# ofsouzap/DistributedMandelbrot

Hardware: AMD Instinct MI355X
Metric: G pixel-iterations/s on 4096^2 tile, max_iter=1000 fp64 (higher is better)
Workload: dtype f64

## Files before the change

distributedmandelbrot_amd/_lib.py:

```python
from __future__ import annotations

import ctypes as C
import importlib.util
import os
import sys

HERE = os.path.dirname(os.path.abspath(__file__))
SO_PATH = os.path.join(HERE, "libmbk_hip.so")

MBK_OK, MBK_ERR_INVALID, MBK_ERR_NO_DEVICE, MBK_ERR_HIP, MBK_ERR_NOMEM, MBK_ERR_NET = range(6)
MBK_WANT_COUNTS = 0x1
MBK_WANT_BYTES = 0x2
MBK_KERNEL_DEFAULT = 0x000
MBK_KERNEL_SIMPLE = 0x100
MBK_KERNEL_ASM = 0x200
MBK_KERNEL_REFILL = 0x300
MBK_KERNEL_GROUP = 0x400
MBK_KERNEL_SCAN = 0x500
KERNELS = {"default": MBK_KERNEL_DEFAULT, "simple": MBK_KERNEL_SIMPLE, "asm": MBK_KERNEL_ASM,
           "refill": MBK_KERNEL_REFILL, "group": MBK_KERNEL_GROUP, "scan": MBK_KERNEL_SCAN}
OPTIONS = {name: i for i, name in enumerate(
    ["order", "waves_per_wg", "group_steps", "exact_steps", "probe_steps", "scan_waves", "scan_xcd_map", "scan_col_period", "heavy_share",
     "rf_livemin", "rf_patience", "rf_batch", "rf_waves", "cycle_detect", "probe_mid", "prepass_overlap", "exact_long", "scan_inline", "wave_limit", "units_min_light", "xcd_balance", "m_late", "h_settled", "classify_wg", "scan_strip", "cycle_window", "spill_first", "spill_lanes", "spill_min_mrd", "spill_min_blocks", "spill_cyc_shift",
     "sure_interior"])}
MBK_PRECISION_F32 = 0x1000
MBK_LAZY_UNIFORM = 0x2000
MBK_DEEP_BLA = 0x8000
MBK_DEEP_XBLA = 0x10000
PRECISIONS = {"f64": 0, "f32": MBK_PRECISION_F32}
MBK_SLOTS = 4
MBK_WORKER_DEPTH = 3
MBK_INFO_SCAN_WG_PER_CU = 100
MBK_INFO_XCD_SHARE = 110
MBK_INFO_SPILL = 130
MBK_CODEC_RAW = 0x00
MBK_CODEC_RLE = 0x01
MBK_CHUNK_DEFINITION = 4096
MBK_CHUNK_BYTES = 4096 * 4096
MBK_ABI_VERSION = 5
MBK_RENDER_BYTES = 0
MBK_RENDER_SMOOTH = 1
MBK_RENDER_DISTANCE = 3
MBK_RENDER_DISTANCE_REL = 4
MBK_RENDER_EQUALIZED = 5
RENDER_SOURCES = {"bytes": MBK_RENDER_BYTES, "smooth": MBK_RENDER_SMOOTH, "distance": MBK_RENDER_DISTANCE,
                  "distance_rel": MBK_RENDER_DISTANCE_REL, "equalized": MBK_RENDER_EQUALIZED}
MBK_HISTOGRAM_MAX_MRD = 1 << 20
# ... 131 lines not shown
    "mbk_view_launch_distance": (C.c_int, [C.c_void_p, C.POINTER(mbk_view), C.c_uint32, C.c_uint32,
                                           C.c_void_p, C.c_void_p, C.c_void_p]),
    "mbk_view_compute_distance": (C.c_int, [C.c_void_p, C.POINTER(mbk_view), C.c_uint32, C.c_uint32,
                                            C.c_void_p, C.c_void_p, C.POINTER(mbk_stats)]),
    "mbk_distance_value_host": (C.c_double, [C.c_double, C.c_double, C.c_int32]),
    "mbk_datachunk_submit": (C.c_int, [C.c_void_p, C.c_int, C.c_uint32, C.c_uint32, C.c_uint32, C.c_uint32,
                                       C.c_void_p, C.c_void_p]),
    "mbk_datachunk_submit_ex": (C.c_int, [C.c_void_p, C.c_int, C.c_uint32, C.c_uint32, C.c_uint32, C.c_uint32,
                                          C.c_void_p, C.c_void_p, C.c_uint32]),
    "mbk_view_submit": (C.c_int, [C.c_void_p, C.c_int, C.POINTER(mbk_view), C.c_uint32, C.c_uint32,
                                  C.c_void_p, C.c_void_p]),
    "mbk_wait": (C.c_int, [C.c_void_p, C.c_int, C.POINTER(mbk_stats)]),
    "mbk_serialize_last": (C.c_int, [C.c_void_p, C.c_void_p, C.c_uint64, C.POINTER(C.c_uint64),
                                     C.POINTER(C.c_uint32)]),
    "mbk_set_option": (C.c_int, [C.c_void_p, C.c_int, C.c_uint32]),
    "mbk_get_option": (C.c_int, [C.c_void_p, C.c_int, C.POINTER(C.c_uint32)]),
    "mbk_quantise_counts": (C.c_int, [C.c_void_p, C.c_void_p, C.c_uint64, C.c_uint32, C.c_void_p]),
    "mbk_units_plan": (C.c_int, [C.c_uint32, C.c_uint32, C.c_uint32, C.c_void_p, C.c_void_p]),
    "mbk_units_lookup": (C.c_int, [C.c_void_p, C.c_uint32, C.c_void_p, C.c_void_p]),
    "mbk_sure_interior_point": (C.c_int, [C.c_double, C.c_double]),
    "mbk_sure_interior_blocks": (C.c_int, [C.POINTER(mbk_view), C.POINTER(C.c_uint64)]),
    "mbk_sure_interior_flag": (C.c_int, [C.POINTER(mbk_view), C.c_uint32, C.c_uint32, C.c_uint32, C.c_uint32,
                                         C.POINTER(C.c_uint32)]),
    "mbk_reduce_counts": (C.c_int, [C.c_void_p, C.c_void_p, C.c_uint64, C.c_uint32, C.c_void_p,
                                    C.POINTER(mbk_stats)]),
    "mbk_worker_run": (C.c_int, [C.c_void_p, C.c_char_p, C.c_uint16, C.c_uint64, C.c_uint32,
                                 C.POINTER(mbk_worker_report)]),
    "mbk_net_set_option": (C.c_int, [C.c_int, C.c_uint32]),
    "mbk_net_get_option": (C.c_int, [C.c_int, C.POINTER(C.c_uint32)]),
    "mbk_feeder_run": (C.c_int, [C.POINTER(mbk_feeder_ops), C.c_char_p, C.c_uint16, C.c_uint64, C.c_uint32,
                                 C.POINTER(mbk_worker_report)]),
    "mbk_deep_orbit_create": (C.c_int, [C.c_char_p, C.c_char_p, C.c_uint32, C.c_uint32, C.POINTER(C.c_void_p)]),
    "mbk_deep_orbit_destroy": (None, [C.c_void_p]),
    "mbk_deep_orbit_info": (C.c_int, [C.c_void_p, C.POINTER(C.c_uint32), C.POINTER(C.c_uint32), C.POINTER(C.c_uint32),
                                      C.POINTER(C.c_uint32)]),
    "mbk_deep_orbit_read": (C.c_int, [C.c_void_p, C.c_void_p, C.c_void_p, C.c_uint64]),
    "mbk_deep_view_launch": (C.c_int, [C.c_void_p, C.c_void_p, C.POINTER(mbk_deep_view), C.c_uint32, C.c_uint32,
                                       C.c_void_p, C.c_void_p, C.c_void_p, C.c_void_p]),
    "mbk_deep_view_compute": (C.c_int, [C.c_void_p, C.c_void_p, C.POINTER(mbk_deep_view), C.c_uint32, C.c_uint32,
                                        C.c_void_p, C.c_void_p, C.c_void_p, C.POINTER(mbk_stats)]),
    "mbk_deep_view_submit": (C.c_int, [C.c_void_p, C.c_int, C.c_void_p, C.POINTER(mbk_deep_view), C.c_uint32, C.c_uint32,
                                       C.c_void_p, C.c_void_p]),
    "mbk_deep_view_launch_distance": (C.c_int, [C.c_void_p, C.c_void_p, C.POINTER(mbk_deep_view), C.c_uint32, C.c_uint32,
                                                C.c_void_p, C.c_void_p, C.c_void_p]),
    "mbk_deep_view_compute_distance": (C.c_int, [C.c_void_p, C.c_void_p, C.POINTER(mbk_deep_view), C.c_uint32, C.c_uint32,
                                                 C.c_void_p, C.c_void_p, C.POINTER(mbk_stats)]),
# ... 287 lines not shown
```

distributedmandelbrot_amd/csrc/mbk_api.hip:

```cpp
#include "../../include/mbk.h"

#include <hip/hip_runtime.h>

#include <cmath>
#include <cstdio>
#include <cstdlib>
#include <algorithm>
#include <cstring>
#include <new>
#include <string>
#include <vector>

#include "mbk_kernels.h"
#include "mbk_refill.h"
#include "mbk_persist.h"
#include "mbk_scan.h"
#include "mbk_units.h"
#include "mbk_spill.h"
#include "mbk_feeder.h"
#include "mbk_deep_orbit.h"
#include "mbk_deep.h"
#include "mbk_deep_bla.h"
#include "mbk_deep_wide.h"
#include "mbk_deep_wide_bla.h"
// ... 371 lines not shown
}

static int get_scratch(mbk_ctx *ctx, hipStream_t stream, StreamScratch **out)
{
    for (StreamScratch &sc : ctx->scratch)
        if (sc.stream == stream) {
            *out = &sc;
            return MBK_OK;
        }
    if (ctx->scratch.size() >= kMaxStreamScratch) {
        MBK_HIP(ctx, hipDeviceSynchronize());
        for (StreamScratch &sc : ctx->scratch) free_scratch(sc);
        ctx->scratch.clear();
    }
    ctx->scratch.emplace_back();
    StreamScratch &sc = ctx->scratch.back();
    sc.stream = stream;
    *out = &sc;
    MBK_HIP(ctx, hipHostMalloc((void **)&sc.h_hint, 2 * sizeof(uint32_t), hipHostMallocDefault));
    sc.h_hint[0] = sc.h_hint[1] = 0xffffffffu;
    return MBK_OK;
}

static void set_window_facts(TileArgs &a, bool f32, bool cyc = true, uint32_t sure_option = 0u);
static void shares_from_fractions(const double *f, uint32_t *cum);
static double window_heavy_share(const TileArgs &a);
static double window_heavy_share(mbk_ctx *ctx, const TileArgs &a);

static void xcd_shares_update(const mbk_ctx *ctx, StreamScratch &sc)
{
    const unsigned long long kMask = 0xffffffffffffull;
    uint32_t first = sc.xcd_issued >= kStampSlots ? sc.xcd_issued - kStampSlots + 1u : 1u;
    first = std::max(first, sc.xcd_consumed + 1u);
    for (uint32_t c = first; c <= sc.xcd_issued; ++c) {
        const volatile unsigned long long *st = sc.h_stamps + (size_t)(c % kStampSlots) * mbk::kStampWords;
        const StreamScratch::SharesUsed &used = sc.xcd_ring[c % kShareRing];
        if (used.seq != c) continue;
        const StreamScratch::SharesUsed &before = sc.xcd_ring[(c - 1u) % kShareRing], &after = sc.xcd_ring[(c + 1u) % kShareRing];
        const bool alone = c > 1u && before.seq == c - 1u && before.switches == used.switches &&
                           (c == sc.xcd_issued ? ctx->stream_switches == used.switches : after.seq == c + 1u && after.switches == used.switches);
        unsigned long long v[mbk::kStampWords];
        bool whole = true;
        for (uint32_t i = 0; i < mbk::kStampWords; ++i) {
            v[i] = st[i];
            whole = whole && (v[i] >> 48) == (c & 0xffffu);
        }
        if (!whole) continue;
// ... 31 lines not shown
{
    uint32_t qtab = 0u;
    if (want_bytes && mrd > 0)
        for (uint32_t c = 1; c <= 4u; ++c)
            qtab |= (uint32_t)(((uint64_t)c * 256u + (uint32_t)mrd - 1u) / (uint32_t)mrd & 0xffu) << (8u * (c - 1u));
    return qtab;
}

struct BlockLaunchPlan {
    uint32_t wpw, by;
    dim3 grid, block;
    uint32_t order_mode, probe_steps;
    bool cyc, units, ordered;
    double unit_share;
};

static BlockLaunchPlan block_launch_plan(mbk_ctx *ctx, TileArgs &a, uint32_t kernel, bool safe, bool f32)
{
    BlockLaunchPlan p;
    p.wpw = ctx->opt[MBK_OPT_WAVES_PER_WG];
    a.blocks_x = (a.ncols + 8u * p.wpw - 1u) / (8u * p.wpw);
    p.by = (a.nrows + 7u) / 8u;
    p.cyc = ctx->opt[MBK_OPT_CYCLE_DETECT] != 0u;
    set_window_facts(a, f32, p.cyc, ctx->opt[MBK_OPT_SURE_INTERIOR]);
    p.grid = dim3(a.blocks_x * p.by);
    p.block = dim3(64u * p.wpw);
    p.order_mode = ctx->opt[MBK_OPT_ORDER];
    p.probe_steps = ctx->opt[MBK_OPT_PROBE_STEPS];
    a.perm_mul = p.order_mode == 1 ? coprime_multiplier(p.grid.x) : 1u;
    a.order = nullptr;
    p.units = p.order_mode == 3 && p.wpw == 1u && kernel == MBK_KERNEL_GROUP && !safe && a.smooth == nullptr &&
              (a.counts || a.bytes) && !(a.bytes && a.quant_wide) && a.blocks_x % 8u == 0u && a.blocks_x <= 2048u &&
              a.fast_bx_end > 0u && a.fast_by_end > 0u && (f32 || ctx->opt[MBK_OPT_GROUP_STEPS] == 16u) &&
              p.grid.x >= 16384u && (uint32_t)a.mrd > 2u * p.probe_steps && p.by <= 0xffffu;
    p.unit_share = 0.0;
    if (p.units) {
        p.unit_share = window_heavy_share(ctx, a);
        p.units = (1.0 - p.unit_share) * 65536.0 >= (double)ctx->opt[MBK_OPT_UNITS_MIN_LIGHT];
    }
    p.ordered = p.order_mode >= 2 && p.grid.x >= 16384u && (uint32_t)a.mrd > 2u * p.probe_steps && a.blocks_x <= 0xffffu && p.by <= 0xffffu;
    return p;
}

struct OrderList {
    StreamScratch *sc = nullptr;
    unsigned k = 0;
    uint32_t *list = nullptr;
// ... 279 lines not shown
        MBK_HIP(ctx, hipEventRecord(ol.sc->ring.ev_done[ol.k], stream));
        ol.sc->ring.done_valid[ol.k] = true;
    }
    if (spill) {
        const int rc = enqueue_spill_second_pass(ctx, a, *spill, p.grid.x, f32, p.cyc, stream);
        if (rc != MBK_OK) return rc;
    }
    ol.whole = true;
    return MBK_OK;
}

static bool window_may_touch_ring(const TileArgs &a, double margin = 1e-6)
{
    const double x0 = axis_value_host(a.re, a.col0), x1 = axis_value_host(a.re, a.col0 + a.ncols - 1u);
    const double y0 = axis_value_host(a.im, a.row0), y1 = axis_value_host(a.im, a.row0 + a.nrows - 1u);
    const double xlo = std::fmin(x0, x1), xhi = std::fmax(x0, x1), ylo = std::fmin(y0, y1), yhi = std::fmax(y0, y1);
    const double dx = (xlo <= 0.0 && 0.0 <= xhi) ? 0.0 : std::fmin(std::fabs(xlo), std::fabs(xhi));
    const double dy = (ylo <= 0.0 && 0.0 <= yhi) ? 0.0 : std::fmin(std::fabs(ylo), std::fabs(yhi));
    const double fx = std::fmax(std::fabs(xlo), std::fabs(xhi)), fy = std::fmax(std::fabs(ylo), std::fabs(yhi));
    const double rmin2 = dx * dx + dy * dy, rmax2 = fx * fx + fy * fy;
    return !(rmax2 < 4.0 - margin || rmin2 > 4.0 + margin);
}

static uint32_t sure_interior_word(const TileArgs &a, bool f32, bool cyc, uint32_t option)
{
    if (option == 0u || f32 || cyc || a.mrd < 65) return 0u;
    if (option == 2u) return 2u;
    if (a.ncols == 0u || a.nrows == 0u) return 0u;
    const double x0 = axis_value_host(a.re, a.col0), x1 = axis_value_host(a.re, a.col0 + a.ncols - 1u);
    const double y0 = axis_value_host(a.im, a.row0), y1 = axis_value_host(a.im, a.row0 + a.nrows - 1u);
    const double xlo = std::fmin(x0, x1), xhi = std::fmax(x0, x1), ylo = std::fmin(y0, y1), yhi = std::fmax(y0, y1);
    if (!(xlo <= 0.4 && xhi >= -1.3 && ylo <= 0.7 && yhi >= -0.7)) return 0u;
    const uint32_t k = 16;
    for (uint32_t j = 0; j < k; ++j) {
        const double ci = axis_value_host(a.im, a.row0 + (uint32_t)(((uint64_t)(2u * j + 1u) * a.nrows) / (2u * k)));
        for (uint32_t i = 0; i < k; ++i)
            if (mbk::sure_interior_point(axis_value_host(a.re, a.col0 + (uint32_t)(((uint64_t)(2u * i + 1u) * a.ncols) / (2u * k))), ci))
                return 1u;
    }
    return 0u;
}

static void set_window_facts(TileArgs &a, bool f32, bool cyc, uint32_t sure_option)
{
    a.sure_interior = sure_interior_word(a, f32, cyc, sure_option);
    a.ring_possible = window_may_touch_ring(a, f32 ? 2e-3 : 1e-6) ? 1u : 0u;
    a.fast_bx_end = a.fast_by_end = 0u;
    if (a.re.step_is_zero || a.im.step_is_zero) return;
    const uint64_t re_n = (uint64_t)a.re.n - (axis_end_is_regular(a.re) ? 0u : 1u), im_n = (uint64_t)a.im.n - (axis_end_is_regular(a.im) ? 0u : 1u);
    const uint64_t cols_ok = std::min<uint64_t>(a.ncols, re_n - std::min<uint64_t>(a.col0, re_n));
    const uint64_t rows_ok = std::min<uint64_t>(a.nrows, im_n - std::min<uint64_t>(a.row0, im_n));
    a.fast_bx_end = (uint32_t)(cols_ok / 8u);
    a.fast_by_end = (uint32_t)(rows_ok / 8u);
}

static int launch_refill(mbk_ctx *ctx, const TileArgs &a, bool safe, hipStream_t stream)
{
    const bool eligible = !safe && a.mrd >= 2 && a.counts != nullptr && !a.re.step_is_zero &&
                          !a.im.step_is_zero && !window_may_touch_ring(a, 1e-6);
    const uint32_t cols_ok = a.re.n > 0 ? std::min<uint64_t>(a.ncols, (uint64_t)(a.re.n - 1u) - std::min<uint64_t>(a.col0, a.re.n - 1u)) : 0u;
    const uint32_t rows_ok = a.im.n > 0 ? std::min<uint64_t>(a.nrows, (uint64_t)(a.im.n - 1u) - std::min<uint64_t>(a.row0, a.im.n - 1u)) : 0u;
    const uint32_t icols = eligible ? (cols_ok / 8u) * 8u : 0u, irows = eligible ? (rows_ok / 8u) * 8u : 0u;
    if (icols == 0 || irows == 0) return launch_blocks(ctx, a, MBK_KERNEL_GROUP, safe, false, stream);

    mbk::PersistArgs q;
    std::memset(&q, 0, sizeof(q));
    q.re_start = a.re.start;
    q.re_step = a.re.step;
// ... 710 lines not shown
}

int mbk_create(int device, mbk_ctx **out)
{
    if (!out) return fail(nullptr, MBK_ERR_INVALID, "out is NULL");
    *out = nullptr;
    int n = 0;
    hipError_t e = hipGetDeviceCount(&n);
    if (e != hipSuccess || n <= 0)
        return fail(nullptr, MBK_ERR_NO_DEVICE,
                    std::string("no HIP device visible (") + hipGetErrorString(e) +
                        "); libmbk_hip has no CPU fallback");
    if (device < 0 || device >= n) return fail(nullptr, MBK_ERR_NO_DEVICE, "device index out of range");
    mbk_ctx *ctx = new (std::nothrow) mbk_ctx();
    if (!ctx) return fail(nullptr, MBK_ERR_NOMEM, "out of host memory");
    ctx->device = device;
    static const uint32_t kDefaults[MBK_OPT_COUNT_] = {
         3u,  1u,  16u,  8u,  32u,
         8u,  1u,  4u,  655u,
         48u,  256u,  1u,  8u,  1u,
         65537u,  1u,  0u,  1u,  0u,
         32768u,  0u,  8u,  6u,  1024u,
         1u,  32u,  256u,  16u,  2048u,  19u,  5u,
         1u};
    std::memcpy(ctx->opt, kDefaults, sizeof(kDefaults));
#define MBK_CREATE_HIP(call)                                                        \
    do {                                                                            \
        hipError_t e2_ = (call);                                                    \
        if (e2_ != hipSuccess) {                                                    \
            fail(nullptr, MBK_ERR_HIP, std::string(#call) + ": " + hipGetErrorString(e2_)); \
            mbk_destroy(ctx);                                                       \
            return MBK_ERR_HIP;                                                     \
        }                                                                           \
    } while (0)
    MBK_CREATE_HIP(hipSetDevice(device));
    MBK_CREATE_HIP(hipGetDeviceProperties(&ctx->prop, device));
    if (std::strncmp(ctx->prop.gcnArchName, "gfx950", 6) != 0) {
        fail(nullptr, MBK_ERR_NO_DEVICE,
             std::string("device is ") + ctx->prop.gcnArchName + ", this library is built for gfx950 only");
        mbk_destroy(ctx);
        return MBK_ERR_NO_DEVICE;
    }
    for (Slot &sl : ctx->s) {
        MBK_CREATE_HIP(hipStreamCreateWithFlags(&sl.stream, hipStreamNonBlocking));
        MBK_CREATE_HIP(hipEventCreate(&sl.ev_k0));
        MBK_CREATE_HIP(hipEventCreate(&sl.ev_k1));
        MBK_CREATE_HIP(hipEventCreate(&sl.ev_c0));
// ... 638 lines not shown
        case MBK_OPT_RF_LIVEMIN: ok = value <= 63u; break;
        case MBK_OPT_RF_PATIENCE: ok = value >= 16u && value <= (1u << 20); break;
        case MBK_OPT_RF_BATCH: ok = value >= 1u && value <= 64u; break;
        case MBK_OPT_RF_WAVES: ok = value >= 1u && value <= 8u; break;
        case MBK_OPT_CYCLE_DETECT: ok = value <= 1u; break;
        case MBK_OPT_PROBE_MID: ok = value >= 2u && value <= 65537u; break;
        case MBK_OPT_PREPASS_OVERLAP: ok = value <= 2u; break;
        case MBK_OPT_CLASSIFY_WG: ok = value >= 64u && value <= 1024u && value % 64u == 0u; break;
        case MBK_OPT_SCAN_STRIP: ok = value <= 1u; break;
        case MBK_OPT_CYCLE_WINDOW: ok = value <= 65536u; break;
        case MBK_OPT_EXACT_LONG: ok = value <= 4096u; break;
        case MBK_OPT_SCAN_INLINE: ok = value <= 1u; break;
        case MBK_OPT_WAVE_LIMIT: ok = value <= 7u; break;
        case MBK_OPT_UNITS_MIN_LIGHT: ok = value <= 65536u; break;
        case MBK_OPT_XCD_BALANCE: ok = value <= 2u; break;
        case MBK_OPT_M_LATE: ok = value <= 65536u; break;
        case MBK_OPT_H_SETTLED: ok = value <= 30u; break;
        case MBK_OPT_SPILL_FIRST: ok = value <= 65536u && value % 32u == 0u; break;
        case MBK_OPT_SPILL_LANES: ok = value >= 1u && value <= 32u; break;
        case MBK_OPT_SPILL_MIN_MRD: ok = true; break;
        case MBK_OPT_SPILL_MIN_BLOCKS: ok = value <= 31u; break;
        case MBK_OPT_SPILL_CYC_SHIFT: ok = value <= 31u; break;
        case MBK_OPT_SURE_INTERIOR: ok = value <= 2u; break;
        default: return fail(ctx, MBK_ERR_INVALID, "unknown MBK_OPT_* selector");
    }
    if (!ok) return fail(ctx, MBK_ERR_INVALID, "option value out of range");
    ctx->opt[option] = value;
    return MBK_OK;
}

int mbk_get_option(mbk_ctx *ctx, int option, uint32_t *value)
{
    if (!ctx || !value) return fail(ctx, MBK_ERR_INVALID, "NULL argument");
    if (option >= MBK_INFO_SCAN_WG_PER_CU && option < MBK_INFO_SCAN_WG_PER_CU + 4) {
        const int k = option - MBK_INFO_SCAN_WG_PER_CU;
        *value = (uint32_t)ctx->scan_occ[k >> 1][k & 1];
        return MBK_OK;
    }
    if (option >= MBK_INFO_XCD_SHARE && option < MBK_INFO_XCD_SHARE + 10) {
        const StreamScratch *best = nullptr;
        for (const StreamScratch &sc : ctx->scratch)
            if (!best || sc.xcd_consumed > best->xcd_consumed) best = &sc;
        const int k = option - MBK_INFO_XCD_SHARE;
        *value = !best ? 0u : k < 8 ? (uint32_t)std::lround(best->xcd_f[k] * 1048576.0) : k == 8 ? best->xcd_consumed : best->xcd_issued;
        return MBK_OK;
    }
// ... 68 lines not shown
            for (uint32_t ly = 0; ly < 8u && all; ++ly) {
                const double ci = (double)(a.row0 + by * 8u + ly) * a.im.step + a.im.start;
                for (uint32_t lx = 0; lx < 8u && all; ++lx)
                    all = mbk::sure_interior_point((double)(a.col0 + bx * 8u + lx) * a.re.step + a.re.start, ci);
            }
            n += all ? 1u : 0u;
        }
    *certified = n;
    return MBK_OK;
}

int mbk_sure_interior_flag(const mbk_view *view, uint32_t mrd, uint32_t flags, uint32_t cycle_detect, uint32_t option, uint32_t *flag)
{
    if (!view || !flag) return fail(nullptr, MBK_ERR_INVALID, "NULL argument");
    if (option > 2u || mrd > 0x7fffffffu) return fail(nullptr, MBK_ERR_INVALID, "option value out of range");
    const bool f32 = (flags & MBK_PRECISION_F32) != 0;
    bool safe = false;
    const int rc = validate_view(nullptr, view, &safe, f32);
    if (rc != MBK_OK) return rc;
    TileArgs a = view_window_args(view);
    a.mrd = (int32_t)mrd;
    set_window_facts(a, f32, cycle_detect != 0u, option);
    *flag = a.sure_interior;
    return MBK_OK;
}

int mbk_quantise_counts(mbk_ctx *ctx, const int32_t *h_counts, uint64_t n, uint32_t mrd, uint8_t *h_bytes)
{
    if (!ctx || !h_counts || !h_bytes) return fail(ctx, MBK_ERR_INVALID, "NULL argument");
    if (mrd == 0 || mrd > 0x7fffffffu) return fail(ctx, MBK_ERR_INVALID, "mrd must be in [1, 2^31)");
    if (n == 0) return MBK_OK;
    if (n > (1ull << 31)) return fail(ctx, MBK_ERR_INVALID, "more than 2^31 counts");
    int rc = sync_begin(ctx);
    if (rc != MBK_OK) return rc;
    Slot &sl = ctx->s[0];
    rc = ensure_buffers(ctx, sl, (size_t)n);
    if (rc != MBK_OK) return rc;
    MBK_HIP(ctx, hipMemcpyAsync(sl.d_counts, h_counts, n * sizeof(int32_t), hipMemcpyHostToDevice, sl.stream));
    hipLaunchKernelGGL(mbk::quantise_kernel, dim3(2048), dim3(256), 0, sl.stream, sl.d_counts, sl.d_bytes, n,
                       (int32_t)mrd, mrd >= (1u << 23) ? 1u : 0u, 1.0 / (double)mrd);
    MBK_HIP(ctx, hipGetLastError());
    MBK_HIP(ctx, hipMemcpyAsync(h_bytes, sl.d_bytes, n, hipMemcpyDeviceToHost, sl.stream));
    MBK_HIP(ctx, hipStreamSynchronize(sl.stream));
    ctx->last_px = 0;
    return MBK_OK;
}
// ... 3357 lines not shown
```

distributedmandelbrot_amd/csrc/mbk_kernels.h:

```cpp
#pragma once

#include <hip/hip_runtime.h>
#include <stdint.h>

namespace mbk {

struct Axis {
    double start;
    double step;
    double last;
    double delta;
    double div;
    uint32_t n;
    uint32_t step_is_zero;
};

constexpr double kSafeImagMin = 0x1p-900;

struct ReduceSlot;

constexpr uint32_t kSpillLevels = 12;

struct TileArgs {
    Axis re, im;
// ... 7 lines not shown
    uint32_t exact_steps_long;
    uint32_t ring_possible;
    uint32_t fast_bx_end, fast_by_end;
    uint32_t perm_mul;
    const uint32_t *order;
    uint32_t ngrid;
    uint32_t order_mid;
    uint32_t unit_stride;
    uint32_t stamp_tag;
    const uint32_t *plan;
    unsigned long long *stamps;
    int32_t *counts;
    uint8_t *bytes;
    double *smooth;
    ReduceSlot *stats;
    uint32_t cyc_window;
    uint32_t spill_first;
    uint32_t spill_lanes;
    uint32_t spill_win_shift;
    void *spill_z;
    uint32_t *spill_meta;
    uint32_t *spill_cnt;
    uint32_t sure_interior;
};

constexpr double kSureMargin = 1e-4;
__host__ __device__ inline bool sure_interior_point(double cr, double ci)
{
    const double ci2 = ci * ci;
    const double x = cr - 0.25;
    const double q = x * x + ci2;
    const bool cardioid = q * (q + x) < 0.25 * ci2 - kSureMargin;
    const double xd = cr + 1.0;
    const bool disk = xd * xd + ci2 < 0.0625 - kSureMargin;
    return cardioid || disk;
}

__device__ __forceinline__ double axis_value(const Axis &a, uint32_t k)
{
    double y;
    if (a.step_is_zero) {
        double q = (double)k / a.div;
        y = q * a.delta;
    } else {
        y = (double)k * a.step;
    }
// ... 125 lines not shown
                 "s_waitcnt lgkmcnt(0)"
                 : "=&s"(v)
                 : "s"(__builtin_amdgcn_kernarg_segment_ptr()), "n"(kOffset)
                 : "memory");
    return v;
}

template <typename T, bool kFmaDouble, int kGroup, bool kCycle = false, bool kSure = false>
__device__ __forceinline__ int32_t block_pixel(const TileArgs &p, uint32_t ucol, uint32_t urow, uint32_t lx, uint32_t ly,
                                               bool long_groups, bool interior = false)
{
    const uint32_t lc = ucol + lx, lr = urow + ly;
    T cr, ci;
    bool ring_test = kGroup != 0 && kFmaDouble;
    if (interior) {
        cr = (T)((double)(p.col0 + lc) * p.re.step + p.re.start);
        ci = (T)((double)(p.row0 + lr) * p.im.step + p.im.start);
        ring_test = ring_test && p.ring_possible != 0u;
    } else {
        if (lc >= p.ncols || lr >= p.nrows) return -1;
        cr = (T)axis_value(p.re, p.col0 + lc);
        ci = (T)axis_value(p.im, p.row0 + lr);
    }
    if constexpr (kSure && kFmaDouble && kGroup == 16 && !kCycle && sizeof(T) == 8) {
        const uint32_t sure = (long_groups && interior) ? kernarg_u32<offsetof(TileArgs, sure_interior)>() : 0u;
        if (sure != 0u) {
            bool take = __ballot(sure_interior_point((double)cr, (double)ci)) == ~0ull;
            if (!take && sure == 2u) take = !(ring_test && wave_touches_ring(cr, ci));
            if (take && escape_steps_sure(cr, ci, kernarg_u32<offsetof(TileArgs, mrd)>() - 1u) == 0ull) {
                const uint32_t pitch = kernarg_u32<offsetof(TileArgs, out_pitch)>();
                const size_t ubase = (size_t)(urow + kernarg_u32<offsetof(TileArgs, out_row0)>()) * pitch + ucol + kernarg_u32<offsetof(TileArgs, out_col0)>();
                const uint32_t loff = ly * pitch + lx;
                if (p.counts) (reinterpret_cast<int32_t *>(kernarg_u64<offsetof(TileArgs, counts)>()) + ubase)[loff] = 0;
                if (p.bytes) (reinterpret_cast<uint8_t *>(kernarg_u64<offsetof(TileArgs, bytes)>()) + ubase)[loff] = (uint8_t)0;
                if (p.smooth) (reinterpret_cast<double *>(kernarg_u64<offsetof(TileArgs, smooth)>()) + ubase)[loff] = 0.0;
                return 0;
            }
        }
    }
    int32_t count;
    T m = 0;
    if (kGroup != 0 && kFmaDouble) {
        bool risky = false;
        if (ring_test) {
            const T c2 = cr * cr + ci * ci;
            const T margin = sizeof(T) == 8 ? (T)1e-9 : (T)1e-3;
            risky = __ballot(__builtin_fabs((double)(c2 - (T)4)) < (double)margin) != 0ull;
        }
        if (risky) {
            count = escape_count_asm<true>(cr, ci, p.mrd, &m);
        } else if (kGroup == 32) {
            count = long_groups ? escape_count_group<32, false>(cr, ci, p.mrd, &m, p.exact_steps_long)
                                : escape_count_group<8, false>(cr, ci, p.mrd, &m, p.exact_steps);
        } else if (kGroup == 16) {
            count = long_groups ? escape_count_group<16, kCycle>(cr, ci, p.mrd, &m, p.exact_steps_long, p.cyc_window)
                                : escape_count_group<8, kCycle>(cr, ci, p.mrd, &m, p.exact_steps, p.cyc_window);
        } else {
            count = escape_count_group<kGroup == 8 ? 8 : 4, kCycle>(cr, ci, p.mrd, &m, p.exact_steps, p.cyc_window);
        }
    } else {
        count = escape_count_asm<kFmaDouble>(cr, ci, p.mrd, &m);
    }
    const size_t ubase = (size_t)(urow + p.out_row0) * p.out_pitch + ucol + p.out_col0;
    const uint32_t loff = ly * p.out_pitch + lx;
    if (p.counts) (p.counts + ubase)[loff] = count;
// ... 393 lines not shown
```

distributedmandelbrot_amd/csrc/mbk_loops.inc:

```
#ifndef MBK_T
#error "define MBK_T and MBK_F before including mbk_loops.inc"
#endif
#define MBK_STEP_HEAD_FMA                                  \
    "v_add_" MBK_F " %[t], %[a], -%[b]\n"                        \
    "v_mul_" MBK_F " %[p], %[zr], %[zi]\n"                       \
    "v_add_" MBK_F " %[zr], %[t], %[cr]\n"                       \
    "v_fma_" MBK_F " %[zi], %[p], 2.0, %[ci]\n"
#define MBK_STEP_HEAD_SAFE                                 \
    "v_add_" MBK_F " %[t], %[a], -%[b]\n"                        \
    "v_add_" MBK_F " %[p], %[zr], %[zr]\n"                       \
    "v_mul_" MBK_F " %[p], %[p], %[zi]\n"                        \
    "v_add_" MBK_F " %[zr], %[t], %[cr]\n"                       \
    "v_add_" MBK_F " %[zi], %[p], %[ci]\n"
#define MBK_STEP_TAIL(ID)                                  \
    "v_mul_" MBK_F " %[a], %[zr], %[zr]\n"                       \
    "v_mul_" MBK_F " %[b], %[zi], %[zi]\n"                       \
    "v_add_" MBK_F " %[m], %[a], %[b]\n"                         \
    "v_cmp_le_" MBK_F " vcc, 4.0, %[m]\n"                        \
    "s_cbranch_vccnz .Lesc" ID "_%=\n"                     \
    ".Lcont" ID "_%=:\n"
#define MBK_ESCAPE(ID, INC)                                \
    ".Lesc" ID "_%=:\n"                                    \
    "s_add_u32 %[k], %[n], " INC "\n"                      \
    "s_and_saveexec_b64 %[tmp], vcc\n"                     \
// ... 264 lines not shown
    "s_cbranch_scc1 .Lgtloop_%=\n"                         \
    "s_branch .Lgdone_%=\n"                                \
    MBK_G_TRIP_A("1", "0")                                 \
    MBK_G_TRIP_B("2", "32")                                \
    MBK_ESCAPE("GT", "1")                                  \
    ".Ldone_%=:\n"                                         \
    ".Lgdone_%=:\n"                                        \
    "s_mov_b64 exec, %[save]\n"                            \
    MBK_G_FIXUP("32")                                      \
    "s_mov_b64 exec, %[save]\n"

#define MBK_G_CYC_INIT                                     \
    "v_mov_" MBK_CYC_MOV " %[szr], %[zr]\n"                \
    "v_mov_" MBK_CYC_MOV " %[szi], %[zi]\n"                \
    "s_mov_b32 %[tc], 0\n"                                 \
    "s_mov_b32 %[win], 1\n"
#define MBK_G_CYC_INIT_W                                   \
    "v_mov_" MBK_CYC_MOV " %[szr], %[zr]\n"                \
    "v_mov_" MBK_CYC_MOV " %[szi], %[zi]\n"                \
    "s_mov_b32 %[tc], 0\n"                                 \
    "s_mov_b32 %[win], %[win0]\n"
#define MBK_G_CYC(ZR, ZI, ID)                              \
    "v_cmp_eq_" MBK_CYC_BITS " vcc, " ZR ", %[szr]\n"      \
    "v_cmp_eq_" MBK_CYC_BITS "_e64 %[tmp2], " ZI ", %[szi]\n" \
    "s_and_b64 vcc, vcc, %[tmp2]\n"                        \
    "s_cbranch_vccnz .Lcyc" ID "_%=\n"                     \
    ".Lcyccont" ID "_%=:\n"                                \
    "s_add_u32 %[tc], %[tc], 1\n"                          \
    "s_cmp_ge_u32 %[tc], %[win]\n"                         \
    "s_cbranch_scc1 .Lcycsave" ID "_%=\n"                  \
    ".Lcycsaved" ID "_%=:\n"
#define MBK_G_CYC_OOL(ZR, ZI, ID)                          \
    ".Lcyc" ID "_%=:\n"                                    \
    "s_and_saveexec_b64 %[tmp], vcc\n"                     \
    "v_mov_b32 %[cnt], -1\n"                               \
    "s_andn2_b64 exec, %[tmp], vcc\n"                      \
    "s_cbranch_scc1 .Lcyccont" ID "_%=\n"                  \
    "s_branch .Lgdone_%=\n"                                \
    ".Lcycsave" ID "_%=:\n"                                \
    "v_mov_" MBK_CYC_MOV " %[szr], " ZR "\n"               \
    "v_mov_" MBK_CYC_MOV " %[szi], " ZI "\n"               \
    "s_mov_b32 %[tc], 0\n"                                 \
    "s_lshr_b32 %[k], %[win], 2\n"                         \
    "s_add_u32 %[k], %[k], 1\n"                            \
    "s_cmp_lt_u32 %[win], %[wcap]\n"                       \
    "s_cselect_b32 %[k], %[k], %[win]\n"                   \
    "s_add_u32 %[win], %[win], %[k]\n"                     \
    "s_branch .Lcycsaved" ID "_%=\n"
#define MBK_G_LOOP8CXI(INIT, FIX) MBK_G_LOOP8X(INIT, MBK_G_CYC("%[zr2]", "%[zi2]", "1"), MBK_G_CYC("%[zr]", "%[zi]", "2"), \
                                               MBK_G_CYC_OOL("%[zr2]", "%[zi2]", "1") MBK_G_CYC_OOL("%[zr]", "%[zi]", "2"), FIX)
#define MBK_G_LOOP8CX(FIX) MBK_G_LOOP8CXI(MBK_G_CYC_INIT, FIX)
#define MBK_G_LOOP8C_W MBK_G_LOOP8CXI(MBK_G_CYC_INIT_W, MBK_G_FIXUP("8"))
#define MBK_G_LOOP16CX(FIX) MBK_G_LOOP16X(MBK_G_CYC_INIT, MBK_G_CYC("%[zrt]", "%[zit]", "M1"), MBK_G_CYC("%[zr2]", "%[zi2]", "1"), \
                                          MBK_G_CYC("%[zrt]", "%[zit]", "M2"), MBK_G_CYC("%[zr]", "%[zi]", "2"), \
                                          MBK_G_CYC_OOL("%[zrt]", "%[zit]", "M1") MBK_G_CYC_OOL("%[zr2]", "%[zi2]", "1") \
                                          MBK_G_CYC_OOL("%[zrt]", "%[zit]", "M2") MBK_G_CYC_OOL("%[zr]", "%[zi]", "2"), FIX)
#define MBK_G_LOOP8C MBK_G_LOOP8CX(MBK_G_FIXUP("8"))
#define MBK_G_LOOP16C MBK_G_LOOP16CX(MBK_G_FIXUP("16"))
// ... 172 lines not shown
    ".Lsone_%=:\n"                                         \
    MBK_G_A2A                                              \
    "s_sub_u32 %[n], %[n], 1\n"                            \
    "s_cmp_lg_u32 %[n], 0\n"                               \
    "s_cbranch_scc1 .Lsone_%=\n"                           \
    ".Lsend_%=:\n"                                         \
    "v_add_" MBK_F " %[m], %[a], %[b]\n"                   \
    "v_cmp_ngt_" MBK_F " vcc, 4.0, %[m]\n"                 \
    "s_mov_b64 %[mask], vcc\n"
__device__ __forceinline__ unsigned long long escape_steps_sure(MBK_T cr, MBK_T ci, uint32_t total)
{
    MBK_T zr = cr, zi = ci;
    MBK_T a = zr * zr, b = zi * zi, m, t, p;
    uint32_t n;
    unsigned long long mask;
    asm volatile(MBK_SURE_LOOP
                 : [zr] "+&v"(zr), [zi] "+&v"(zi), [a] "+&v"(a), [b] "+&v"(b), [m] "=&v"(m), [t] "=&v"(t), [p] "=&v"(p),
                   [n] "=&s"(n), [mask] "=&s"(mask)
                 : [cr] "v"(cr), [ci] "v"(ci), [total] "s"(total)
                 : "vcc", "scc");
    return mask;
}

template <bool kFmaDouble>
__device__ __forceinline__ int32_t escape_count_asm_from(MBK_T z0r, MBK_T z0i, MBK_T cr, MBK_T ci, int32_t mrd, MBK_T *m_out = nullptr)
{
    MBK_T zr = z0r, zi = z0i;
    MBK_T a = zr * zr, b = zi * zi, m = 0;
    int32_t cnt = 0;
    escape_steps_asm<kFmaDouble>(cr, ci, zr, zi, a, b, m, cnt, 0u, mrd > 1 ? (uint32_t)mrd - 1u : 0u);
    if (m_out) *m_out = m;
    return cnt;
}

template <int kGroup = 8, bool kCycle = false>
__device__ __forceinline__ int32_t escape_count_group_from(MBK_T z0r, MBK_T z0i, MBK_T cr, MBK_T ci, int32_t mrd, MBK_T *m_out = nullptr,
                                                           uint32_t kExactSteps = 8, uint32_t cyc_wcap = 32u)
{
    MBK_T zr = z0r, zi = z0i;
    MBK_T a = zr * zr, b = zi * zi, m = 0;
    int32_t cnt = 0;
    const uint32_t total = mrd > 1 ? (uint32_t)mrd - 1u : 0u;
    const uint32_t first = total < kExactSteps ? total : kExactSteps;
    escape_steps_asm<true>(cr, ci, zr, zi, a, b, m, cnt, 0u, first);
    if (cnt == 0 && total > first) escape_steps_tail<kGroup, kCycle>(cr, ci, zr, zi, a, b, m, cnt, first, total, cyc_wcap);
    if (m_out) *m_out = m;
// ... 224 lines not shown
```

include/mbk.h:

```cpp
#ifndef MBK_H
#define MBK_H

#include <stdint.h>

#ifdef __cplusplus
extern "C" {
#endif

#define MBK_ABI_VERSION 5

#define MBK_CHUNK_DEFINITION 4096u
#define MBK_CHUNK_BYTES (4096u * 4096u)

enum mbk_status {
    MBK_OK = 0,
    MBK_ERR_INVALID = 1,
    MBK_ERR_NO_DEVICE = 2,
    MBK_ERR_HIP = 3,
    MBK_ERR_NOMEM = 4,
    MBK_ERR_NET = 5
};

#define MBK_WANT_COUNTS 0x1u
#define MBK_WANT_BYTES 0x2u
// ... 463 lines not shown
    MBK_OPT_RF_LIVEMIN,
    MBK_OPT_RF_PATIENCE,
    MBK_OPT_RF_BATCH,
    MBK_OPT_RF_WAVES,
    MBK_OPT_CYCLE_DETECT,
    MBK_OPT_PROBE_MID,
    MBK_OPT_PREPASS_OVERLAP,
    MBK_OPT_EXACT_LONG,
    MBK_OPT_SCAN_INLINE,
    MBK_OPT_WAVE_LIMIT,
    MBK_OPT_UNITS_MIN_LIGHT,
    MBK_OPT_XCD_BALANCE,
    MBK_OPT_M_LATE,
    MBK_OPT_H_SETTLED,
    MBK_OPT_CLASSIFY_WG,
    MBK_OPT_SCAN_STRIP,
    MBK_OPT_CYCLE_WINDOW,
    MBK_OPT_SPILL_FIRST,
    MBK_OPT_SPILL_LANES,
    MBK_OPT_SPILL_MIN_MRD,
    MBK_OPT_SPILL_MIN_BLOCKS,
    MBK_OPT_SPILL_CYC_SHIFT,
    MBK_OPT_SURE_INTERIOR,
    MBK_OPT_COUNT_
};
#define MBK_INFO_SCAN_WG_PER_CU 100
#define MBK_INFO_XCD_SHARE 110
#define MBK_INFO_SPILL 130
int mbk_set_option(mbk_ctx *ctx, int option, uint32_t value);
int mbk_get_option(mbk_ctx *ctx, int option, uint32_t *value);

int mbk_units_plan(uint32_t n_h, uint32_t n_v, uint32_t n_m, const double *fractions, uint32_t *plan);
int mbk_units_lookup(const uint32_t *plan, uint32_t id, uint32_t *list, uint32_t *index);

int mbk_sure_interior_point(double cr, double ci);
int mbk_sure_interior_blocks(const mbk_view *view, uint64_t *certified);
int mbk_sure_interior_flag(const mbk_view *view, uint32_t mrd, uint32_t flags, uint32_t cycle_detect, uint32_t option,
                           uint32_t *flag);

int mbk_quantise_counts(mbk_ctx *ctx, const int32_t *h_counts, uint64_t n, uint32_t mrd, uint8_t *h_bytes);

int mbk_reduce_counts(mbk_ctx *ctx, const int32_t *d_counts, uint64_t n, uint32_t mrd,
                      void *hip_stream, mbk_stats *stats);

typedef struct mbk_worker_report {
    uint64_t leased;
    uint64_t accepted;
    uint64_t rejected;
    uint64_t resets;
    uint64_t uniform_tiles;
    uint64_t pixel_iterations;
    double kernel_ms_sum;
    double seconds;
    uint64_t net_retries;
} mbk_worker_report;
int mbk_worker_run(mbk_ctx *ctx, const char *addr, uint16_t port, uint64_t max_tiles, uint32_t senders,
                   mbk_worker_report *report);

enum mbk_net_option {
    MBK_NET_MAX_CONNECTIONS = 0,
    MBK_NET_CONNECT_TIMEOUT_MS = 1,
// ... 27 lines not shown
```

Baseline: 5462.

## Add sure-interior certification path for cycle-detect kernels

```diff
diff --git a/distributedmandelbrot_amd/_lib.py b/distributedmandelbrot_amd/_lib.py
--- a/distributedmandelbrot_amd/_lib.py
+++ b/distributedmandelbrot_amd/_lib.py
@@ -22,7 +22,7 @@
 OPTIONS = {name: i for i, name in enumerate(
     ["order", "waves_per_wg", "group_steps", "exact_steps", "probe_steps", "scan_waves", "scan_xcd_map", "scan_col_period", "heavy_share",
      "rf_livemin", "rf_patience", "rf_batch", "rf_waves", "cycle_detect", "probe_mid", "prepass_overlap", "exact_long", "scan_inline", "wave_limit", "units_min_light", "xcd_balance", "m_late", "h_settled", "classify_wg", "scan_strip", "cycle_window", "spill_first", "spill_lanes", "spill_min_mrd", "spill_min_blocks", "spill_cyc_shift",
-     "sure_interior"])}
+     "sure_interior", "sure_cycle"])}
 MBK_PRECISION_F32 = 0x1000
 MBK_LAZY_UNIFORM = 0x2000
 MBK_DEEP_BLA = 0x8000
@@ -200,6 +200,8 @@
     "mbk_sure_interior_blocks": (C.c_int, [C.POINTER(mbk_view), C.POINTER(C.c_uint64)]),
     "mbk_sure_interior_flag": (C.c_int, [C.POINTER(mbk_view), C.c_uint32, C.c_uint32, C.c_uint32, C.c_uint32,
                                          C.POINTER(C.c_uint32)]),
+    "mbk_sure_cycle_flag": (C.c_int, [C.POINTER(mbk_view), C.c_uint32, C.c_uint32, C.c_uint32, C.c_uint32,
+                                      C.POINTER(C.c_uint32)]),
     "mbk_reduce_counts": (C.c_int, [C.c_void_p, C.c_void_p, C.c_uint64, C.c_uint32, C.c_void_p,
                                     C.POINTER(mbk_stats)]),
     "mbk_worker_run": (C.c_int, [C.c_void_p, C.c_char_p, C.c_uint16, C.c_uint64, C.c_uint32,
diff --git a/distributedmandelbrot_amd/csrc/mbk_api.hip b/distributedmandelbrot_amd/csrc/mbk_api.hip
--- a/distributedmandelbrot_amd/csrc/mbk_api.hip
+++ b/distributedmandelbrot_amd/csrc/mbk_api.hip
@@ -417,7 +417,7 @@
     return MBK_OK;
 }
 
-static void set_window_facts(TileArgs &a, bool f32, bool cyc = true, uint32_t sure_option = 0u);
+static void set_window_facts(TileArgs &a, bool f32, bool cyc = true, uint32_t sure_option = 0u, uint32_t sure_cycle_option = 0u);
 static void shares_from_fractions(const double *f, uint32_t *cum);
 static double window_heavy_share(const TileArgs &a);
 static double window_heavy_share(mbk_ctx *ctx, const TileArgs &a);
@@ -495,7 +495,7 @@
     a.blocks_x = (a.ncols + 8u * p.wpw - 1u) / (8u * p.wpw);
     p.by = (a.nrows + 7u) / 8u;
     p.cyc = ctx->opt[MBK_OPT_CYCLE_DETECT] != 0u;
-    set_window_facts(a, f32, p.cyc, ctx->opt[MBK_OPT_SURE_INTERIOR]);
+    set_window_facts(a, f32, p.cyc, ctx->opt[MBK_OPT_SURE_INTERIOR], ctx->opt[MBK_OPT_SURE_CYCLE]);
     p.grid = dim3(a.blocks_x * p.by);
     p.block = dim3(64u * p.wpw);
     p.order_mode = ctx->opt[MBK_OPT_ORDER];
@@ -821,9 +821,9 @@
     return !(rmax2 < 4.0 - margin || rmin2 > 4.0 + margin);
 }
 
-static uint32_t sure_interior_word(const TileArgs &a, bool f32, bool cyc, uint32_t option)
-{
-    if (option == 0u || f32 || cyc || a.mrd < 65) return 0u;
+static uint32_t sure_word(const TileArgs &a, bool f32, uint32_t option)
+{
+    if (option == 0u || f32 || a.mrd < 65) return 0u;
     if (option == 2u) return 2u;
     if (a.ncols == 0u || a.nrows == 0u) return 0u;
     const double x0 = axis_value_host(a.re, a.col0), x1 = axis_value_host(a.re, a.col0 + a.ncols - 1u);
@@ -839,10 +839,13 @@
     }
     return 0u;
 }
-
-static void set_window_facts(TileArgs &a, bool f32, bool cyc, uint32_t sure_option)
+static uint32_t sure_interior_word(const TileArgs &a, bool f32, bool cyc, uint32_t option) { return cyc ? 0u : sure_word(a, f32, option); }
+static uint32_t sure_cycle_word(const TileArgs &a, bool f32, bool cyc, uint32_t option) { return cyc ? sure_word(a, f32, option) : 0u; }
+
+static void set_window_facts(TileArgs &a, bool f32, bool cyc, uint32_t sure_option, uint32_t sure_cycle_option)
 {
     a.sure_interior = sure_interior_word(a, f32, cyc, sure_option);
+    a.sure_cycle = sure_cycle_word(a, f32, cyc, sure_cycle_option);
     a.ring_possible = window_may_touch_ring(a, f32 ? 2e-3 : 1e-6) ? 1u : 0u;
     a.fast_bx_end = a.fast_by_end = 0u;
     if (a.re.step_is_zero || a.im.step_is_zero) return;
@@ -1599,7 +1602,7 @@
          65537u,  1u,  0u,  1u,  0u,
          32768u,  0u,  8u,  6u,  1024u,
          1u,  32u,  256u,  16u,  2048u,  19u,  5u,
-         1u};
+         1u,  1u};
     std::memcpy(ctx->opt, kDefaults, sizeof(kDefaults));
 #define MBK_CREATE_HIP(call)                                                        \
     do {                                                                            \
@@ -2284,6 +2287,7 @@
         case MBK_OPT_SPILL_MIN_BLOCKS: ok = value <= 31u; break;
         case MBK_OPT_SPILL_CYC_SHIFT: ok = value <= 31u; break;
         case MBK_OPT_SURE_INTERIOR: ok = value <= 2u; break;
+        case MBK_OPT_SURE_CYCLE: ok = value <= 2u; break;
         default: return fail(ctx, MBK_ERR_INVALID, "unknown MBK_OPT_* selector");
     }
     if (!ok) return fail(ctx, MBK_ERR_INVALID, "option value out of range");
@@ -2398,6 +2402,21 @@
     a.mrd = (int32_t)mrd;
     set_window_facts(a, f32, cycle_detect != 0u, option);
     *flag = a.sure_interior;
+    return MBK_OK;
+}
+
+int mbk_sure_cycle_flag(const mbk_view *view, uint32_t mrd, uint32_t flags, uint32_t cycle_detect, uint32_t option, uint32_t *flag)
+{
+    if (!view || !flag) return fail(nullptr, MBK_ERR_INVALID, "NULL argument");
+    if (option > 2u || mrd > 0x7fffffffu) return fail(nullptr, MBK_ERR_INVALID, "option value out of range");
+    const bool f32 = (flags & MBK_PRECISION_F32) != 0;
+    bool safe = false;
+    const int rc = validate_view(nullptr, view, &safe, f32);
+    if (rc != MBK_OK) return rc;
+    TileArgs a = view_window_args(view);
+    a.mrd = (int32_t)mrd;
+    set_window_facts(a, f32, cycle_detect != 0u, 0u, option);
+    *flag = a.sure_cycle;
     return MBK_OK;
 }
 
diff --git a/distributedmandelbrot_amd/csrc/mbk_kernels.h b/distributedmandelbrot_amd/csrc/mbk_kernels.h
--- a/distributedmandelbrot_amd/csrc/mbk_kernels.h
+++ b/distributedmandelbrot_amd/csrc/mbk_kernels.h
@@ -53,6 +53,7 @@
     uint32_t *spill_meta;
     uint32_t *spill_cnt;
     uint32_t sure_interior;
+    uint32_t sure_cycle;
 };
 
 constexpr double kSureMargin = 1e-4;
@@ -224,12 +225,16 @@
         cr = (T)axis_value(p.re, p.col0 + lc);
         ci = (T)axis_value(p.im, p.row0 + lr);
     }
-    if constexpr (kSure && kFmaDouble && kGroup == 16 && !kCycle && sizeof(T) == 8) {
-        const uint32_t sure = (long_groups && interior) ? kernarg_u32<offsetof(TileArgs, sure_interior)>() : 0u;
+    bool certified = false;
+    if constexpr (kSure && kFmaDouble && kGroup == 16 && sizeof(T) == 8) {
+        uint32_t sure = 0u;
+        if (long_groups && interior) sure = kCycle ? kernarg_u32<offsetof(TileArgs, sure_cycle)>() : kernarg_u32<offsetof(TileArgs, sure_interior)>();
         if (sure != 0u) {
             bool take = __ballot(sure_interior_point((double)cr, (double)ci)) == ~0ull;
             if (!take && sure == 2u) take = !(ring_test && wave_touches_ring(cr, ci));
-            if (take && escape_steps_sure(cr, ci, kernarg_u32<offsetof(TileArgs, mrd)>() - 1u) == 0ull) {
+            if constexpr (kCycle) {
+                certified = take && escape_steps_sure_cycle(cr, ci, kernarg_u32<offsetof(TileArgs, mrd)>() - 1u, p.cyc_window) == 0ull;
+            } else if (take && escape_steps_sure(cr, ci, kernarg_u32<offsetof(TileArgs, mrd)>() - 1u) == 0ull) {
                 const uint32_t pitch = kernarg_u32<offsetof(TileArgs, out_pitch)>();
                 const size_t ubase = (size_t)(urow + kernarg_u32<offsetof(TileArgs, out_row0)>()) * pitch + ucol + kernarg_u32<offsetof(TileArgs, out_col0)>();
                 const uint32_t loff = ly * pitch + lx;
@@ -242,7 +247,9 @@
     }
     int32_t count;
     T m = 0;
-    if (kGroup != 0 && kFmaDouble) {
+    if (certified) {
+        count = 0;
+    } else if (kGroup != 0 && kFmaDouble) {
         bool risky = false;
         if (ring_test) {
             const T c2 = cr * cr + ci * ci;
diff --git a/distributedmandelbrot_amd/csrc/mbk_loops.inc b/distributedmandelbrot_amd/csrc/mbk_loops.inc
--- a/distributedmandelbrot_amd/csrc/mbk_loops.inc
+++ b/distributedmandelbrot_amd/csrc/mbk_loops.inc
@@ -310,18 +310,20 @@
     "s_mov_b32 %[win], %[win0]\n"
 #define MBK_G_CYC(ZR, ZI, ID)                              \
     "v_cmp_eq_" MBK_CYC_BITS " vcc, " ZR ", %[szr]\n"      \
-    "v_cmp_eq_" MBK_CYC_BITS "_e64 %[tmp2], " ZI ", %[szi]\n" \
-    "s_and_b64 vcc, vcc, %[tmp2]\n"                        \
     "s_cbranch_vccnz .Lcyc" ID "_%=\n"                     \
     ".Lcyccont" ID "_%=:\n"                                \
     "s_add_u32 %[tc], %[tc], 1\n"                          \
     "s_cmp_ge_u32 %[tc], %[win]\n"                         \
     "s_cbranch_scc1 .Lcycsave" ID "_%=\n"                  \
     ".Lcycsaved" ID "_%=:\n"
-#define MBK_G_CYC_OOL(ZR, ZI, ID)                          \
+#define MBK_G_CYC_OOL(ZR, ZI, ID) MBK_G_CYC_OOL_X(ZR, ZI, ID, "v_mov_b32 %[cnt], -1\n")
+#define MBK_G_CYC_OOL_X(ZR, ZI, ID, RETIRE)                \
     ".Lcyc" ID "_%=:\n"                                    \
+    "v_cmp_eq_" MBK_CYC_BITS "_e64 %[tmp2], " ZI ", %[szi]\n" \
+    "s_and_b64 vcc, vcc, %[tmp2]\n"                        \
+    "s_cbranch_scc0 .Lcyccont" ID "_%=\n"                  \
     "s_and_saveexec_b64 %[tmp], vcc\n"                     \
-    "v_mov_b32 %[cnt], -1\n"                               \
+    RETIRE                                                 \
     "s_andn2_b64 exec, %[tmp], vcc\n"                      \
     "s_cbranch_scc1 .Lcyccont" ID "_%=\n"                  \
     "s_branch .Lgdone_%=\n"                                \
@@ -540,6 +542,58 @@
     return mask;
 }
 
+#define MBK_G_A2A8 MBK_G_A2A4 MBK_G_A2A4
+#define MBK_G_CYC_OOL_S(ID) MBK_G_CYC_OOL_X("%[zr]", "%[zi]", ID, "v_add_" MBK_F " %[t], %[a], %[b]\n")
+#define MBK_SURE_CYC_LOOP                                  \
+    "s_mov_b64 %[save], exec\n"                            \
+    MBK_G_CYC_INIT                                         \
+    "s_lshr_b32 %[n], %[total], 5\n"                       \
+    "s_cmp_eq_u32 %[n], 0\n"                               \
+    "s_cbranch_scc1 .Lsrem_%=\n"                           \
+    ".Lsmain_%=:\n"                                        \
+    MBK_G_A2A8 MBK_G_CYC("%[zr]", "%[zi]", "1")            \
+    MBK_G_A2A8 MBK_G_CYC("%[zr]", "%[zi]", "2")            \
+    MBK_G_A2A8 MBK_G_CYC("%[zr]", "%[zi]", "3")            \
+    MBK_G_A2A8 MBK_G_CYC("%[zr]", "%[zi]", "4")            \
+    "s_sub_u32 %[n], %[n], 1\n"                            \
+    "s_cmp_lg_u32 %[n], 0\n"                               \
+    "s_cbranch_scc1 .Lsmain_%=\n"                          \
+    ".Lsrem_%=:\n"                                         \
+    "s_and_b32 %[n], %[total], 31\n"                       \
+    "s_cmp_eq_u32 %[n], 0\n"                               \
+    "s_cbranch_scc1 .Lsend_%=\n"                           \
+    ".Lsone_%=:\n"                                         \
+    MBK_G_A2A                                              \
+    "s_sub_u32 %[n], %[n], 1\n"                            \
+    "s_cmp_lg_u32 %[n], 0\n"                               \
+    "s_cbranch_scc1 .Lsone_%=\n"                           \
+    ".Lsend_%=:\n"                                         \
+    "v_add_" MBK_F " %[t], %[a], %[b]\n"                   \
+    ".Lgdone_%=:\n"                                        \
+    "s_mov_b64 exec, %[save]\n"                            \
+    "v_cmp_ngt_" MBK_F " vcc, 4.0, %[t]\n"                 \
+    "s_mov_b64 %[mask], vcc\n"                             \
+    "s_branch .Lsout_%=\n"                                 \
+    MBK_G_CYC_OOL_S("1") MBK_G_CYC_OOL_S("2") MBK_G_CYC_OOL_S("3") MBK_G_CYC_OOL_S("4") \
+    ".Lsout_%=:\n"
+__device__ __forceinline__ unsigned long long escape_steps_sure_cycle(MBK_T cr, MBK_T ci, uint32_t total, uint32_t cyc_wcap)
+{
+    MBK_T zr = cr, zi = ci;
+    MBK_T a = zr * zr, b = zi * zi, t, p, szr, szi;
+    uint32_t n, k, tc, win;
+    unsigned long long save, tmp, tmp2, mask;
+    asm volatile(MBK_SURE_CYC_LOOP
+                 : [zr] "+&v"(zr), [zi] "+&v"(zi), [a] "+&v"(a), [b] "+&v"(b), [t] "=&v"(t), [p] "=&v"(p), [szr] "=&v"(szr), [szi] "=&v"(szi),
+                   [n] "=&s"(n), [k] "=&s"(k), [tc] "=&s"(tc), [win] "=&s"(win),
+                   [save] "=&s"(save), [tmp] "=&s"(tmp), [tmp2] "=&s"(tmp2), [mask] "=&s"(mask)
+                 : [cr] "v"(cr), [ci] "v"(ci), [total] "s"(total), [wcap] "s"(cyc_wcap)
+                 : "vcc", "scc");
+    return mask;
+}
+#undef MBK_G_A2A8
+#undef MBK_G_CYC_OOL_S
+#undef MBK_SURE_CYC_LOOP
+
 template <bool kFmaDouble>
 __device__ __forceinline__ int32_t escape_count_asm_from(MBK_T z0r, MBK_T z0i, MBK_T cr, MBK_T ci, int32_t mrd, MBK_T *m_out = nullptr)
 {
diff --git a/include/mbk.h b/include/mbk.h
--- a/include/mbk.h
+++ b/include/mbk.h
@@ -509,6 +509,7 @@
     MBK_OPT_SPILL_MIN_BLOCKS,
     MBK_OPT_SPILL_CYC_SHIFT,
     MBK_OPT_SURE_INTERIOR,
+    MBK_OPT_SURE_CYCLE,
     MBK_OPT_COUNT_
 };
 #define MBK_INFO_SCAN_WG_PER_CU 100
@@ -524,6 +525,8 @@
 int mbk_sure_interior_blocks(const mbk_view *view, uint64_t *certified);
 int mbk_sure_interior_flag(const mbk_view *view, uint32_t mrd, uint32_t flags, uint32_t cycle_detect, uint32_t option,
                            uint32_t *flag);
+int mbk_sure_cycle_flag(const mbk_view *view, uint32_t mrd, uint32_t flags, uint32_t cycle_detect, uint32_t option,
+                        uint32_t *flag);
 
 int mbk_quantise_counts(mbk_ctx *ctx, const int32_t *h_counts, uint64_t n, uint32_t mrd, uint8_t *h_bytes);
 
```

Result: no change. 5466 (median of 2 runs) (+0.1%).
